# Ezreal11/EaBNet

Hardware: AMD Instinct MI355X
Metric: enhanced frames/sec (16 kHz, 8-mic) at 1/2/4/8 MI355X; RTF per utterance (higher is better)
Workload: dtype f32; 1 GPU; BASELINE configs[1]/[2]: batch of 16 four-second 8-mic 16 kHz utterances per GPU, wave -> STFT+compress -> EaBNet.forward, inference, full hand-written HIP path; batch_per_gpu=16, global_batch=16, mics=8, frames_per_utt=401, freq_bins=161, parallelism=dp1 (independent shards, no collective), pipeline_depth=3

## Files before the change

eabnet_amd/csrc/conv_gemm.hip:

```cpp
#include "device.h"
#include <type_traits>

#define CG_THREADS 256

#define CG_PLAIN 0
#define CG_GLU 1
#define CG_DUAL 2
#define CG_PH2 3
#define CG_XFC 128

#define CG_PMAX 352

template <int MI, int NI, int KU, int MODE, bool PATCH>
struct CgSmem {
    static constexpr int BM = 64 * MI, BN = 64 * NI, LDK = 16 * KU + 4;
    static constexpr int NA = MODE == CG_DUAL ? 2 : 1;
    static constexpr int ATILE = BM * LDK;
    float a[PATCH ? CG_PMAX * LDK : NA * 2 * ATILE];
    float b[2][BN * LDK];
    float xft[2][CG_XFC][2];
    float xsl[2][CG_XFC];
    int dt[EAB_MAX_TAPS];
    int ioff[EAB_MAX_TAPS];
    int last;
};

__device__ __forceinline__ void cg_merge(float& n, float& mean, float& m2, float nb, float meanb, float m2b) {
    const float nt = n + nb;
    if (nt > 0.0f) {
        const float delta = meanb - mean;
        const float fb = nb / nt;
        mean = fmaf(delta, fb, mean);
        m2 = m2 + m2b + delta * delta * n * fb;
    }
    n = nt;
}

template <int MI, int NI, int KU, int MODE, int XF, bool VEC, int PREC, bool PATCH, bool WIDE = false>
__global__ __launch_bounds__(CG_THREADS, (MI == 2 && NI == 2 && KU == 1 && MODE == CG_GLU) ? 3 : (MODE == CG_PH2 ? 2 : 1)) void conv_gemm_kernel(const eab_conv_desc d) {
    static_assert(MODE != CG_PH2 || (PATCH && NI == 2), "phase-pair form: patch pipeline, one column block per phase and wave");
    static_assert(!PATCH || (KU == 1 && MODE != CG_DUAL && VEC), "patch mode: one unit per stage, single transform");
    constexpr bool H3 = PREC == EAB_PREC_F16X3;
    constexpr bool BF = PREC == EAB_PREC_BF16;
    constexpr bool PH2 = MODE == CG_PH2;
    constexpr bool GLU = MODE != CG_PLAIN;
    constexpr bool DUAL = MODE == CG_DUAL;
    using Smem = CgSmem<MI, NI, KU, MODE, PATCH>;
    constexpr int BM = Smem::BM, BN = Smem::BN, LDK = Smem::LDK;
    __shared__ __attribute__((aligned(16))) Smem sm;

    const int tid = threadIdx.x;
    const int lane = tid & 63, wave = tid >> 6;
    const int wm = wave >> 1, wn = wave & 1;
    const int li = lane & 31, lh = lane >> 5;

    const int t_lo = d.win.pos ? *d.win.pos : 0;
    int t_hi = d.win.pos ? (t_lo + d.win.count < d.T ? t_lo + d.win.count : d.T) : d.T;
    const int tiles_per_b = ((d.win.pos ? d.win.count : d.T) * d.No + BM - 1) / BM;
    unsigned vblk = blockIdx.x;
    if (gridDim.x >= 64) {
        const unsigned G = gridDim.x, G8 = G >> 3, rem = G & 7, xcd = vblk & 7, idx = vblk >> 3;
        vblk = xcd * G8 + (xcd < rem ? xcd : rem) + idx;
    }
    const int b = (int)(vblk / (unsigned)tiles_per_b);
    const int tile = (int)vblk - b * tiles_per_b;
    if (d.win.lens) t_hi = min(t_hi, d.win.lens[b]);
    const int Q = t_hi * d.No;
    const int q0 = t_lo * d.No + tile * BM;
    const int n_blk = blockIdx.y * BN;
    const float inv_no = 1.0f / (float)d.No;

#pragma unroll
    for (int j = 0; j < EAB_MAX_TAPS; ++j)
        if (tid == j) {
            sm.dt[j] = d.dt[j];
            sm.ioff[j] = d.ioff[j];
        }

    if (XF != EAB_XF_NONE) {
        const int k = tid >> 7, c = tid & (CG_XFC - 1);
        const int Ck = (k == 0 || DUAL) ? d.C0 : d.C1;
        const float* xfk = k == 0 ? d.xf0 : d.xf1;
        const float* slk = k == 0 ? d.slope0 : d.slope1;
        float sc = 1.0f, sh = 0.0f, sl = 1.0f;
        if (c < Ck) {
            if (d.fin_stats && k < d.fin_nsets) {
                const float* gm = k == 0 ? d.fin_gamma0 : d.fin_gamma1;
                const float* bt = k == 0 ? d.fin_beta0 : d.fin_beta1;
                double sn = 0.0, sm = 0.0, sq = 0.0;
                for (int t = 0; t < d.fin_tiles; ++t) {
                    const f32x4 v = *reinterpret_cast<const f32x4*>(
                        &d.fin_stats[((((size_t)b * d.fin_tiles + t) * d.fin_nsets + k) * d.C0 + c) * 4]);
                    const double n = (double)v[0], mu = (double)v[1];
                    sn += n;
                    sm = fma(n, mu, sm);
                    sq += fma(n * mu, mu, (double)v[2]);
                }
                const double mean = sn > 0.0 ? sm / sn : 0.0;
                double var = sn > 0.0 ? sq / sn - mean * mean : 0.0;
                if (var < 0.0) var = 0.0;
                const double scale = (double)gm[c] / sqrt(var + (double)d.fin_eps);
                sc = (float)scale;
                sh = (float)((double)bt[c] - mean * scale);
                sl = slk[c];
            } else if (xfk) {
                const float2 v = *reinterpret_cast<const float2*>(&xfk[((size_t)b * Ck + c) * 2]);
                sc = v.x;
                sh = v.y;
                sl = slk[c];
            }
        }
        sm.xft[k][c][0] = sc;
        sm.xft[k][c][1] = sh;
        sm.xsl[k][c] = sl;
    }

    const int Ctot = d.C0 + d.C1;
    const int UPT = (Ctot + 15) >> 4;
    const int NU = d.ntaps * UPT;
    static_assert(!WIDE || (PREC == EAB_PREC_BF16 && KU == 1 && VEC && !PATCH && XF == EAB_XF_NONE && MODE != CG_DUAL), "WIDE: see above");
    constexpr bool w0 = WIDE, w1 = WIDE;
    const int NS = (w0 || w1) ? d.ntaps * ((w0 ? d.C0 >> 5 : (d.C0 + 15) >> 4) + (d.C1 > 0 ? (w1 ? d.C1 >> 5 : (d.C1 + 15) >> 4) : 0))
                              : (NU + KU - 1) / KU;

    constexpr unsigned esz0 = WIDE ? 2u : 4u, esz1 = WIDE ? 2u : 4u;
    const unsigned bytes0 = (unsigned)d.T * d.Fin * d.C0 * esz0;
    const unsigned bytes1 = (unsigned)d.T * d.Fin * d.C1 * esz1;
    const __amdgpu_buffer_rsrc_t rs0 = __builtin_amdgcn_make_buffer_rsrc(
        const_cast<char*>(reinterpret_cast<const char*>(d.src0)) + (size_t)b * bytes0, 0, bytes0, 0x00020000);
    const __amdgpu_buffer_rsrc_t rs1 = __builtin_amdgcn_make_buffer_rsrc(
        const_cast<char*>(reinterpret_cast<const char*>(d.src1 ? d.src1 : d.src0)) + (d.src1 ? (size_t)b * bytes1 : 0), 0,
        d.src1 ? bytes1 : 0u, 0x00020000);

    const int srow = tid >> 2;
    const int skq = tid & 3;
    int a_t[MI], a_f0[MI], a_tf[MI];
    bool a_ok[MI];
#pragma unroll
    for (int p = 0; p < MI; ++p) {
        const int q = q0 + srow + 64 * p;
        a_ok[p] = q < Q;
        const int t = a_ok[p] ? eab_div(q, d.No, inv_no) : 0;
        const int o = a_ok[p] ? q - t * d.No : 0;
        a_t[p] = t;
        a_f0[p] = o * d.istride;
        a_tf[p] = t * d.Fin + o * d.istride;
    }
    const float* wrow[NI];
#pragma unroll
    for (int p = 0; p < NI; ++p) wrow[p] = d.w + (size_t)(n_blk + srow + 64 * p) * d.Kpad + skq * 4;

    f32x16 acc[MI][NI];
#pragma unroll
    for (int mi = 0; mi < MI; ++mi)
#pragma unroll
        for (int ni = 0; ni < NI; ++ni)
#pragma unroll
            for (int r = 0; r < 16; ++r) acc[mi][ni][r] = 0.0f;

    auto lds_barrier = [] { asm volatile("s_waitcnt lgkmcnt(0)\n\ts_barrier" ::: "memory"); };

    __syncthreads();

    if (q0 < Q) {
    if constexpr (PATCH) {
        constexpr int PP = (CG_PMAX + 63) / 64;
        int dt_min = 0, io_min = 0, io_max = 0;
#pragma unroll
        for (int j = 0; j < EAB_MAX_TAPS; ++j)
            if (j < d.ntaps) {
                dt_min = d.dt[j] < dt_min ? d.dt[j] : dt_min;
                io_min = d.ioff[j] < io_min ? d.ioff[j] : io_min;
                io_max = d.ioff[j] > io_max ? d.ioff[j] : io_max;
            }
        const int halo_lo = -io_min;
        const int hi_need = (d.No - 1) * d.istride + io_max - (d.Fin - 1);
        const int Fp = d.Fin + halo_lo + (hi_need > 0 ? hi_need : 0);
        const float inv_fp = 1.0f / (float)Fp;
        const int t_first = eab_div(q0, d.No, inv_no);
        const int t_last = eab_div((q0 + BM < Q ? q0 + BM : (Q > q0 ? Q : q0 + 1)) - 1, d.No, inv_no);
        const int P = (t_last - t_first + 1 - dt_min) * Fp;

        int p_tf[PP];
        bool p_ok[PP];
#pragma unroll
        for (int pp = 0; pp < PP; ++pp) {
            const int pidx = srow + 64 * pp;
            const int tr = eab_div(pidx, Fp, inv_fp);
            const int t_in = t_first + dt_min + tr, fi = pidx - tr * Fp - halo_lo;
            p_ok[pp] = pidx < P && t_in >= 0 && t_in < d.T && fi >= 0 && fi < d.Fin;
            p_tf[pp] = t_in * d.Fin + fi;
        }
        int fa[MI];
#pragma unroll
        for (int mi = 0; mi < MI; ++mi) {
            int q = q0 + (wm * MI + mi) * 32 + li;
            q = q < Q ? q : (Q > q0 ? Q - 1 : q0);
            const int t = eab_div(q, d.No, inv_no), o = q - t * d.No;
            fa[mi] = ((t - t_first - dt_min) * Fp + o * d.istride + halo_lo) * LDK + 4 * lh;
        }
        const int b_base = (wn * NI * 32 + li) * LDK + 4 * lh;

        f32x4 rp[PP];
        f32x4 rbw0[NI], rbw1[NI];
        int p_tc = 0;
        auto patch_fetch = [&](int chunk) {
            const int c0 = chunk << 4;
            const bool second = (d.C1 > 0) && (c0 >= d.C0);
            const int Cs = second ? d.C1 : d.C0;
            const int c = (second ? c0 - d.C0 : c0) + skq * 4;
            const bool cok = c < Cs;
            p_tc = ((second ? 1 : 0) << 8) | (cok ? c : 0);
#pragma unroll
            for (int pp = 0; pp < PP; ++pp) {
                const unsigned off = (p_ok[pp] && cok) ? (unsigned)((p_tf[pp] * Cs + c) * 4) : EAB_OOB;
                const u32x4 v = second ? __builtin_amdgcn_raw_buffer_load_b128(rs1, off, 0, 0)
                                       : __builtin_amdgcn_raw_buffer_load_b128(rs0, off, 0, 0);
                rp[pp] = __builtin_bit_cast(f32x4, v);
            }
        };
        auto patch_stash = [&]() {
            f32x4 sh01, sh23, sl;
            if (XF != EAB_XF_NONE) {
                const int cc = p_tc & 0xFF, tb = p_tc >> 8;
                sh01 = *reinterpret_cast<const f32x4*>(&sm.xft[tb][cc][0]);
                sh23 = *reinterpret_cast<const f32x4*>(&sm.xft[tb][cc + 2][0]);
                sl = *reinterpret_cast<const f32x4*>(&sm.xsl[tb][cc]);
            }
#pragma unroll
            for (int pp = 0; pp < PP; ++pp) {
                const int pidx = srow + 64 * pp;
                if (pidx >= CG_PMAX) continue;
                f32x4 v = rp[pp];
                if (XF != EAB_XF_NONE) {
                    const f32x4 x = eab_xform<XF>(v, sh01, sh23, sl);
                    v = p_ok[pp] ? x : f32x4{0.f, 0.f, 0.f, 0.f};
                }
                float* arow = &sm.a[pidx * LDK];
                if (BF) {
                    *reinterpret_cast<uint2*>(reinterpret_cast<char*>(arow) + skq * 8) = make_uint2(eab_bf2(v[0], v[1]), eab_bf2(v[2], v[3]));
                } else if (H3) {
                    unsigned h01, l01, h23, l23;
                    eab_split2(v[0], v[1], h01, l01);
                    eab_split2(v[2], v[3], h23, l23);
                    *reinterpret_cast<uint2*>(reinterpret_cast<char*>(arow) + skq * 8) = make_uint2(h01, h23);
                    *reinterpret_cast<uint2*>(reinterpret_cast<char*>(arow) + 32 + skq * 8) = make_uint2(l01, l23);
                } else {
                    *reinterpret_cast<f32x4*>(arow + skq * 4) = v;
                }
            }
        };
        auto b_fetch = [&](int u, f32x4 (&rbw)[NI]) {
            const int uu = u < NU ? u : 0;
#pragma unroll
            for (int p = 0; p < NI; ++p) rbw[p] = *reinterpret_cast<const f32x4*>(wrow[p] + (size_t)uu * 16);
        };
        auto b_stash = [&](int buf, const f32x4 (&rbw)[NI]) {
#pragma unroll
            for (int p = 0; p < NI; ++p) {
                float* brow = &sm.b[buf][(srow + 64 * p) * LDK];
                if (BF) {
                    *reinterpret_cast<uint2*>(reinterpret_cast<char*>(brow) + skq * 8) =
                        make_uint2(eab_bf2(rbw[p][0], rbw[p][1]), eab_bf2(rbw[p][2], rbw[p][3]));
                } else if (H3) {
                    const u32x4 w = __builtin_bit_cast(u32x4, rbw[p]);
                    *reinterpret_cast<uint2*>(reinterpret_cast<char*>(brow) + skq * 8) = make_uint2(w[0], w[1]);
                    *reinterpret_cast<uint2*>(reinterpret_cast<char*>(brow) + 32 + skq * 8) = make_uint2(w[2], w[3]);
                } else {
                    *reinterpret_cast<f32x4*>(brow + skq * 4) = rbw[p];
                }
            }
        };
        auto pcompute_n = [&](int cur, int tap, auto ne_c) {
            constexpr int NE = decltype(ne_c)::value;
            const int toff = (sm.dt[tap] * Fp + sm.ioff[tap]) * LDK;
            if (BF) {
                bf16x8 ab[MI], bb[NE];
#pragma unroll
                for (int mi = 0; mi < MI; ++mi) ab[mi] = *reinterpret_cast<const bf16x8*>(&sm.a[fa[mi] + toff]);
#pragma unroll
                for (int ni = 0; ni < NE; ++ni) bb[ni] = *reinterpret_cast<const bf16x8*>(&sm.b[cur][b_base + ni * 32 * LDK]);
#pragma unroll
                for (int mi = 0; mi < MI; ++mi)
#pragma unroll
                    for (int ni = 0; ni < NE; ++ni)
                        acc[mi][ni] = __builtin_amdgcn_mfma_f32_32x32x16_bf16(ab[mi], bb[ni], acc[mi][ni], 0, 0, 0);
            } else if (H3) {
                h16x8 ah[MI], al[MI], bh[NE], bl[NE];
#pragma unroll
                for (int mi = 0; mi < MI; ++mi) {
                    const char* pa = reinterpret_cast<const char*>(&sm.a[fa[mi] + toff]);
                    ah[mi] = *reinterpret_cast<const h16x8*>(pa);
                    al[mi] = *reinterpret_cast<const h16x8*>(pa + 32);
                }
#pragma unroll
                for (int ni = 0; ni < NE; ++ni) {
                    const char* pb = reinterpret_cast<const char*>(&sm.b[cur][b_base + ni * 32 * LDK]);
                    bh[ni] = *reinterpret_cast<const h16x8*>(pb);
                    bl[ni] = *reinterpret_cast<const h16x8*>(pb + 32);
                }
#pragma unroll
                for (int mi = 0; mi < MI; ++mi)
#pragma unroll
                    for (int ni = 0; ni < NE; ++ni) {
                        acc[mi][ni] = __builtin_amdgcn_mfma_f32_32x32x16_f16(al[mi], bh[ni], acc[mi][ni], 0, 0, 0);
                        acc[mi][ni] = __builtin_amdgcn_mfma_f32_32x32x16_f16(ah[mi], bl[ni], acc[mi][ni], 0, 0, 0);
                        acc[mi][ni] = __builtin_amdgcn_mfma_f32_32x32x16_f16(ah[mi], bh[ni], acc[mi][ni], 0, 0, 0);
                    }
            } else {
#pragma unroll
                for (int g = 0; g < 2; ++g) {
                    f32x4 af[MI], bf[NE];
#pragma unroll
                    for (int mi = 0; mi < MI; ++mi) af[mi] = *reinterpret_cast<const f32x4*>(&sm.a[fa[mi] + toff + g * 8]);
#pragma unroll
                    for (int ni = 0; ni < NE; ++ni)
                        bf[ni] = *reinterpret_cast<const f32x4*>(&sm.b[cur][b_base + ni * 32 * LDK + g * 8]);
#pragma unroll
                    for (int k = 0; k < 4; ++k)
#pragma unroll
                        for (int mi = 0; mi < MI; ++mi)
#pragma unroll
                            for (int ni = 0; ni < NE; ++ni)
                                acc[mi][ni] = __builtin_amdgcn_mfma_f32_32x32x2f32(af[mi][k], bf[ni][k], acc[mi][ni], 0, 0, 0);
                }
            }
        };
        const unsigned p2mask = PH2 ? (unsigned)d.p2_mask1 : ~0u;
        auto pcompute = [&](int cur, int tap) {
            if (PH2 && !((p2mask >> tap) & 1u)) pcompute_n(cur, tap, std::integral_constant<int, 1>{});
            else pcompute_n(cur, tap, std::integral_constant<int, NI>{});
        };

        patch_fetch(0);
        b_fetch(0, rbw0);
        patch_stash();
        b_stash(0, rbw0);
        b_fetch(1, rbw0);
        b_fetch(2, rbw1);
        lds_barrier();
        const int pre = d.ntaps >= 3 ? d.ntaps - 3 : 0;
        int chunk = 0, tap = 0;
        auto stage = [&](int u, int cur, f32x4 (&rnext)[NI]) {
            if (tap == pre && chunk + 1 < UPT) patch_fetch(chunk + 1);
            pcompute(cur, tap);
            if (u + 1 < NU) b_stash(cur ^ 1, rnext);
            b_fetch(u + 3, rnext);
            if (tap == d.ntaps - 1 && chunk + 1 < UPT) {
                lds_barrier();
                patch_stash();
            }
            lds_barrier();
            if (++tap == d.ntaps) { tap = 0; ++chunk; }
        };
        for (int u = 0; u < NU; u += 2) {
            stage(u, 0, rbw0);
            if (u + 1 < NU) stage(u + 1, 1, rbw1);
        }
        __syncthreads();
    } else {
    struct Stage {
        f32x4 ra[KU][MI], rb[KU][NI];
        f32x4 rb2[BF ? NI : 1];
        int r_tc[KU];
        bool st_ok[KU][MI];
    };
    Stage sa;

    bool tap_ok[MI];
    unsigned tap_b0[MI], tap_b1[MI];
#pragma unroll
    for (int p = 0; p < MI; ++p) {
        tap_ok[p] = false;
        tap_b0[p] = tap_b1[p] = 0u;
    }
    int g_tap = -1, g_c0 = 0, g_w = 16;
    constexpr bool LEAN = KU == 1 && VEC && !DUAL;
    const __amdgpu_buffer_rsrc_t rsw = __builtin_amdgcn_make_buffer_rsrc(const_cast<float*>(d.w), 0, (unsigned)d.N * d.Kpad * 4u, 0x00020000);
    unsigned w_off[NI];
#pragma unroll
    for (int p = 0; p < NI; ++p) w_off[p] = (unsigned)((n_blk + srow + 64 * p) * d.Kpad + skq * 4) * 4u;
    auto fetch = [&](int stage, Stage& rg) {
        if constexpr (LEAN) {
            if (stage == 0) {
                g_tap = 0;
                g_c0 = 0;
            } else {
                g_c0 += g_w;
                if (g_c0 >= (UPT << 4)) {
                    g_c0 = 0;
                    ++g_tap;
                }
            }
            if (g_c0 == 0) {
                const int dt = sm.dt[g_tap], io = sm.ioff[g_tap];
#pragma unroll
                for (int p = 0; p < MI; ++p) {
                    const int tt = a_t[p] + dt, fi = a_f0[p] + io;
                    tap_ok[p] = a_ok[p] && tt >= 0 && tt < d.T && fi >= 0 && fi < d.Fin;
                    const unsigned pos = (unsigned)(a_tf[p] + dt * d.Fin + io);
                    tap_b0[p] = (pos * (unsigned)d.C0 + (unsigned)(skq * (w0 ? 8 : 4))) * esz0;
                    tap_b1[p] = (pos * (unsigned)d.C1 + (unsigned)(skq * (w1 ? 8 : 4))) * esz1;
                }
            }
            const bool second = (d.C1 > 0) && (g_c0 >= d.C0);
            const int Cs = second ? d.C1 : d.C0;
            const int cu = second ? g_c0 - d.C0 : g_c0;
            constexpr bool half = WIDE;
            g_w = half ? 32 : 16;
            const bool cok = cu + skq * (half ? 8 : 4) < Cs;
            const int k0 = g_tap * (UPT << 4) + g_c0;
#pragma unroll
            for (int p = 0; p < MI; ++p) {
                const bool ok = tap_ok[p] && cok;
                rg.st_ok[0][p] = ok;
                const unsigned off = ok ? (second ? tap_b1[p] : tap_b0[p]) : EAB_OOB;
                const u32x4 v = second ? __builtin_amdgcn_raw_buffer_load_b128(rs1, off, cu * (half ? 2 : 4), 0)
                                       : __builtin_amdgcn_raw_buffer_load_b128(rs0, off, cu * (half ? 2 : 4), 0);
                rg.ra[0][p] = __builtin_bit_cast(f32x4, v);
            }
            rg.r_tc[0] = ((half ? 1 : 0) << 9) | ((second ? 1 : 0) << 8) | cu;
#pragma unroll
            for (int p = 0; p < NI; ++p) {
                if constexpr (WIDE) {
                    rg.rb[0][p] = __builtin_bit_cast(f32x4, __builtin_amdgcn_raw_buffer_load_b128(rsw, w_off[p] + skq * 16, k0 * 4, 0));
                    if constexpr (BF)
                        rg.rb2[p] = __builtin_bit_cast(f32x4, __builtin_amdgcn_raw_buffer_load_b128(rsw, w_off[p] + skq * 16, k0 * 4 + 16, 0));
                } else {
                    rg.rb[0][p] = __builtin_bit_cast(f32x4, __builtin_amdgcn_raw_buffer_load_b128(rsw, w_off[p], k0 * 4, 0));
                }
            }
            return;
        }
#pragma unroll
        for (int ku = 0; ku < KU; ++ku) {
            const int u = stage * KU + ku;
            const bool live = u < NU;
            if (u == 0) {
                g_tap = 0;
                g_c0 = 0;
            } else if (live) {
                g_c0 += 16;
                if (g_c0 >= (UPT << 4)) {
                    g_c0 = 0;
                    ++g_tap;
                }
            }
            const int uu = live ? u : 0;
            const int c0 = live ? g_c0 : 0;
            if (live && c0 == 0) {
                const int dt = sm.dt[g_tap], io = sm.ioff[g_tap];
#pragma unroll
                for (int p = 0; p < MI; ++p) {
                    const int tt = a_t[p] + dt, fi = a_f0[p] + io;
                    tap_ok[p] = a_ok[p] && tt >= 0 && tt < d.T && fi >= 0 && fi < d.Fin;
                    const unsigned pos = (unsigned)(a_tf[p] + dt * d.Fin + io);
                    tap_b0[p] = pos * (unsigned)(d.C0 * 4);
                    tap_b1[p] = pos * (unsigned)(d.C1 * 4);
                }
            }
            const bool second = (d.C1 > 0) && (c0 >= d.C0);
            const int Cs = second ? d.C1 : d.C0;
            const int c = (second ? c0 - d.C0 : c0) + skq * 4;
            const bool cok = live && (c < Cs);
#pragma unroll
            for (int p = 0; p < MI; ++p) {
                const bool ok = tap_ok[p] && cok;
                rg.st_ok[ku][p] = ok;
                const unsigned off = ok ? (second ? tap_b1[p] : tap_b0[p]) + (unsigned)(c * 4) : EAB_OOB;
                if (VEC) {
                    const u32x4 v = second ? __builtin_amdgcn_raw_buffer_load_b128(rs1, off, 0, 0)
                                           : __builtin_amdgcn_raw_buffer_load_b128(rs0, off, 0, 0);
                    rg.ra[ku][p] = __builtin_bit_cast(f32x4, v);
                } else {
#pragma unroll
                    for (int j = 0; j < 4; ++j) {
                        const unsigned oj = (ok && c + j < Cs) ? off + 4u * j : EAB_OOB;
                        const unsigned v = second ? __builtin_amdgcn_raw_buffer_load_b32(rs1, oj, 0, 0)
                                                  : __builtin_amdgcn_raw_buffer_load_b32(rs0, oj, 0, 0);
                        rg.ra[ku][p][j] = __builtin_bit_cast(float, v);
                    }
                }
            }
            rg.r_tc[ku] = ((second ? 1 : 0) << 8) | (cok ? c : 0);
#pragma unroll
            for (int p = 0; p < NI; ++p) {
                rg.rb[ku][p] = *reinterpret_cast<const f32x4*>(wrow[p] + (size_t)uu * 16);
                if (!live) rg.rb[ku][p] = f32x4{0.f, 0.f, 0.f, 0.f};
            }
        }
    };

    auto stash = [&](int buf, const Stage& rg) {
#pragma unroll
        for (int ku = 0; ku < KU; ++ku) {
            f32x4 sh01[2], sh23[2], sl[2];
            bool all_ok = false;
            if (XF != EAB_XF_NONE) {
                if constexpr (LEAN) {
                    const int tb = (rg.r_tc[ku] >> 8) & 1, cu = rg.r_tc[ku] & 0xFF;
                    const char* px = reinterpret_cast<const char*>(&sm.xft[0][skq * 4][0]) + (tb * CG_XFC + cu) * 8;
                    const char* ps = reinterpret_cast<const char*>(&sm.xsl[0][skq * 4]) + (tb * CG_XFC + cu) * 4;
                    sh01[0] = *reinterpret_cast<const f32x4*>(px);
                    sh23[0] = *reinterpret_cast<const f32x4*>(px + 16);
                    sl[0] = *reinterpret_cast<const f32x4*>(ps);
                    bool ok_all = true;
#pragma unroll
                    for (int p = 0; p < MI; ++p) ok_all = ok_all && rg.st_ok[ku][p];
                    all_ok = __builtin_amdgcn_ballot_w64(ok_all) == __builtin_amdgcn_ballot_w64(true);
                } else {
                const int cc = rg.r_tc[ku] & 0xFF;
#pragma unroll
                for (int k = 0; k < (DUAL ? 2 : 1); ++k) {
// ... 24 lines not shown
                        else
                            *reinterpret_cast<uint2*>(reinterpret_cast<char*>(arow) + skq * 8) = make_uint2(eab_bf2(v[0], v[1]), eab_bf2(v[2], v[3]));
                    } else if (H3) {
                        unsigned h01, l01, h23, l23;
                        eab_split2(v[0], v[1], h01, l01);
                        eab_split2(v[2], v[3], h23, l23);
                        *reinterpret_cast<uint2*>(reinterpret_cast<char*>(arow) + skq * 8) = make_uint2(h01, h23);
                        *reinterpret_cast<uint2*>(reinterpret_cast<char*>(arow) + 32 + skq * 8) = make_uint2(l01, l23);
                    } else {
                        *reinterpret_cast<f32x4*>(arow + skq * 4) = v;
                    }
                }
            }
#pragma unroll
            for (int p = 0; p < NI; ++p) {
                float* brow = &sm.b[buf][(srow + 64 * p) * LDK + ku * 16];
                if (BF) {
                    if constexpr (WIDE) {
                        const f32x4 r0 = rg.rb[ku][p], r1 = rg.rb2[BF ? p : 0];
                        *reinterpret_cast<u32x4*>(reinterpret_cast<char*>(brow) + skq * 16) =
                            u32x4{eab_bf2(r0[0], r0[1]), eab_bf2(r0[2], r0[3]), eab_bf2(r1[0], r1[1]), eab_bf2(r1[2], r1[3])};
                    } else {
                        *reinterpret_cast<uint2*>(reinterpret_cast<char*>(brow) + skq * 8) =
                            make_uint2(eab_bf2(rg.rb[ku][p][0], rg.rb[ku][p][1]), eab_bf2(rg.rb[ku][p][2], rg.rb[ku][p][3]));
                    }
                } else if (H3) {
                    const u32x4 w = __builtin_bit_cast(u32x4, rg.rb[ku][p]);
                    *reinterpret_cast<uint2*>(reinterpret_cast<char*>(brow) + skq * 8) = make_uint2(w[0], w[1]);
                    *reinterpret_cast<uint2*>(reinterpret_cast<char*>(brow) + 32 + skq * 8) = make_uint2(w[2], w[3]);
                } else {
                    *reinterpret_cast<f32x4*>(brow + skq * 4) = rg.rb[ku][p];
                }
            }
        }
    };

    fetch(0, sa);
    stash(0, sa);
    lds_barrier();

    const int a_base = (wm * MI * 32 + li) * LDK + 4 * lh;
    const int b_base = (wn * NI * 32 + li) * LDK + 4 * lh;

    auto compute = [&](int cur) {
        if (BF) {
#pragma unroll
            for (int ku = 0; ku < KU; ++ku) {
                bf16x8 ab[Smem::NA][MI], bb[NI];
#pragma unroll
                for (int k = 0; k < Smem::NA; ++k)
#pragma unroll
                    for (int mi = 0; mi < MI; ++mi)
                        ab[k][mi] = *reinterpret_cast<const bf16x8*>(&sm.a[(k * 2 + cur) * Smem::ATILE + a_base + mi * 32 * LDK + ku * 16]);
#pragma unroll
                for (int ni = 0; ni < NI; ++ni) bb[ni] = *reinterpret_cast<const bf16x8*>(&sm.b[cur][b_base + ni * 32 * LDK + ku * 16]);
#pragma unroll
                for (int mi = 0; mi < MI; ++mi)
#pragma unroll
                    for (int ni = 0; ni < NI; ++ni)
                        acc[mi][ni] = __builtin_amdgcn_mfma_f32_32x32x16_bf16(ab[DUAL ? ni : 0][mi], bb[ni], acc[mi][ni], 0, 0, 0);
            }
            if constexpr (WIDE) {
                bf16x8 ab[MI], bb[NI];
#pragma unroll
                for (int mi = 0; mi < MI; ++mi) ab[mi] = *reinterpret_cast<const bf16x8*>(&sm.a[cur * Smem::ATILE + a_base + mi * 32 * LDK + 8]);
#pragma unroll
                for (int ni = 0; ni < NI; ++ni) bb[ni] = *reinterpret_cast<const bf16x8*>(&sm.b[cur][b_base + ni * 32 * LDK + 8]);
#pragma unroll
                for (int mi = 0; mi < MI; ++mi)
#pragma unroll
                    for (int ni = 0; ni < NI; ++ni)
                        acc[mi][ni] = __builtin_amdgcn_mfma_f32_32x32x16_bf16(ab[mi], bb[ni], acc[mi][ni], 0, 0, 0);
            }
        } else if (H3) {
#pragma unroll
            for (int ku = 0; ku < KU; ++ku) {
                h16x8 ah[Smem::NA][MI], al[Smem::NA][MI], bh[NI], bl[NI];
#pragma unroll
                for (int k = 0; k < Smem::NA; ++k)
#pragma unroll
                    for (int mi = 0; mi < MI; ++mi) {
                        const char* pa = reinterpret_cast<const char*>(&sm.a[(k * 2 + cur) * Smem::ATILE + a_base + mi * 32 * LDK + ku * 16]);
                        ah[k][mi] = *reinterpret_cast<const h16x8*>(pa);
                        al[k][mi] = *reinterpret_cast<const h16x8*>(pa + 32);
                    }
#pragma unroll
                for (int ni = 0; ni < NI; ++ni) {
                    const char* pb = reinterpret_cast<const char*>(&sm.b[cur][b_base + ni * 32 * LDK + ku * 16]);
                    bh[ni] = *reinterpret_cast<const h16x8*>(pb);
                    bl[ni] = *reinterpret_cast<const h16x8*>(pb + 32);
                }
#pragma unroll
                for (int mi = 0; mi < MI; ++mi)
#pragma unroll
                    for (int ni = 0; ni < NI; ++ni) {
                        const int ka = DUAL ? ni : 0;
                        acc[mi][ni] = __builtin_amdgcn_mfma_f32_32x32x16_f16(al[ka][mi], bh[ni], acc[mi][ni], 0, 0, 0);
                        acc[mi][ni] = __builtin_amdgcn_mfma_f32_32x32x16_f16(ah[ka][mi], bl[ni], acc[mi][ni], 0, 0, 0);
                        acc[mi][ni] = __builtin_amdgcn_mfma_f32_32x32x16_f16(ah[ka][mi], bh[ni], acc[mi][ni], 0, 0, 0);
                    }
            }
        } else {
#pragma unroll
        for (int g = 0; g < 2 * KU; ++g) {
            f32x4 af[Smem::NA][MI], bf[NI];
#pragma unroll
            for (int k = 0; k < Smem::NA; ++k)
#pragma unroll
                for (int mi = 0; mi < MI; ++mi)
                    af[k][mi] = *reinterpret_cast<const f32x4*>(&sm.a[(k * 2 + cur) * Smem::ATILE + a_base + mi * 32 * LDK + g * 8]);
#pragma unroll
            for (int ni = 0; ni < NI; ++ni)
                bf[ni] = *reinterpret_cast<const f32x4*>(&sm.b[cur][b_base + ni * 32 * LDK + g * 8]);
#pragma unroll
            for (int k = 0; k < 4; ++k)
#pragma unroll
                for (int mi = 0; mi < MI; ++mi)
#pragma unroll
                    for (int ni = 0; ni < NI; ++ni)
                        acc[mi][ni] = __builtin_amdgcn_mfma_f32_32x32x2f32(af[DUAL ? ni : 0][mi][k], bf[ni][k],
                                                                           acc[mi][ni], 0, 0, 0);
        }
        }
    };
    constexpr bool PF2 = MI * NI <= 2 && KU == 1 && MODE == CG_PLAIN;
    if constexpr (PF2) {
        Stage sb;
        if (NS > 1) fetch(1, sb);
        for (int s = 0; s < NS; s += 2) {
            if (s + 2 < NS) fetch(s + 2, sa);
            compute(0);
            if (s + 1 < NS) stash(1, sb);
            lds_barrier();
            if (s + 1 < NS) {
                if (s + 3 < NS) fetch(s + 3, sb);
                compute(1);
                if (s + 2 < NS) stash(0, sa);
                lds_barrier();
            }
        }
    } else {
    for (int s = 0; s < NS; ++s) {
        const int cur = s & 1;
        if (s + 1 < NS) fetch(s + 1, sa);
        compute(cur);
        if (s + 1 < NS) stash(cur ^ 1, sa);
        lds_barrier();
    }
    }

    }
    }

    constexpr int NC = GLU ? 1 : NI;
    const int Cout = d.Cout;
    int ch[NC];
    float bias_v[NI];
#pragma unroll
    for (int ni = 0; ni < NI; ++ni) {
        const int n = n_blk + (wn * NI + ni) * 32 + li;
        bias_v[ni] = d.bias ? d.bias[n] : 0.0f;
    }
    if (GLU) {
        ch[0] = (n_blk >> 1) + wn * 32 + li;
    } else {
#pragma unroll
        for (int ni = 0; ni < NI; ++ni) ch[ni] = n_blk + (wn * NI + ni) * 32 + li;
    }
    float st_slope[2][NC];
#pragma unroll
    for (int s = 0; s < 2; ++s)
#pragma unroll
        for (int c = 0; c < NC; ++c) {
            const float* sp = s == 0 ? d.stat_slope0 : d.stat_slope1;
            st_slope[s][c] = (d.stats && s < d.nsets && sp) ? sp[ch[c]] : 1.0f;
        }
    float skk[2][NC], ssum[2][NC], ssq[2][NC];
    float scount = 0.0f;
#pragma unroll
    for (int s = 0; s < 2; ++s)
#pragma unroll
        for (int c = 0; c < NC; ++c) skk[s][c] = ssum[s][c] = ssq[s][c] = 0.0f;
    const bool two_sets = d.nsets == 2;
    const unsigned out_bytes = (unsigned)d.T * d.Fout * Cout * 4u;
    const size_t out_b = (size_t)b * d.T * d.Fout * Cout;
    const bool need_aux = d.epi == EAB_EPI_MULSIG || d.epi == EAB_EPI_ADD;
    const __amdgpu_buffer_rsrc_t r_dst = __builtin_amdgcn_make_buffer_rsrc(d.dst + out_b, 0, out_bytes, 0x00020000);
    const __amdgpu_buffer_rsrc_t r_aux = __builtin_amdgcn_make_buffer_rsrc(
        const_cast<float*>(need_aux ? d.aux + out_b : d.dst + out_b), 0, need_aux ? out_bytes : 0u, 0x00020000);
    const __amdgpu_buffer_rsrc_t r_acc = __builtin_amdgcn_make_buffer_rsrc(
        d.dst_acc ? d.dst_acc + out_b : d.dst + out_b, 0, d.dst_acc ? out_bytes : 0u, 0x00020000);

    const unsigned row_bytes = (unsigned)(d.Fout * Cout) * 4u, step_bytes = (unsigned)(d.ostride * Cout) * 4u;
    const unsigned phase_bytes = (unsigned)(d.ophase * Cout) * 4u;
    if constexpr (PH2) {
        const float a = st_slope[0][0];
        const float k0 = eab_prelu(acc[0][0][0] + bias_v[0], a);
        const unsigned chan_bytes = (unsigned)Cout * 4u;
        float su = 0.0f, sq = 0.0f, cnt = 0.0f;
        auto ph2_loop = [&](auto full_c) {
            constexpr bool FULL = decltype(full_c)::value;
#pragma unroll
            for (int mi = 0; mi < MI; ++mi) {
#pragma unroll
                for (int r4 = 0; r4 < 4; ++r4) {
                    const int qg = q0 + (wm * MI + mi) * 32 + 8 * r4 + 4 * lh;
                    const int t = eab_div((FULL || qg < Q) ? qg : 0, d.No, inv_no);
                    int o = ((FULL || qg < Q) ? qg : 0) - t * d.No;
                    unsigned row_start = (unsigned)t * row_bytes;
                    unsigned cur = row_start + (unsigned)o * step_bytes;
#pragma unroll
                    for (int j = 0; j < 4; ++j) {
                        const int r = 4 * r4 + j;
                        const bool ok0 = FULL || qg + j < Q;
                        const bool ok1 = ok0 && 2 * o + 1 < d.Fout;
                        const float v0 = acc[mi][0][r] + bias_v[0], v1 = acc[mi][1][r] + bias_v[1];
                        const unsigned o0 = cur + 4u * ch[0];
                        __builtin_amdgcn_raw_buffer_store_b32(__builtin_bit_cast(unsigned, v0), r_dst, ok0 ? o0 : EAB_OOB, 0, 0);
                        __builtin_amdgcn_raw_buffer_store_b32(__builtin_bit_cast(unsigned, v1), r_dst, ok1 ? o0 + chan_bytes : EAB_OOB, 0, 0);
                        const float e0 = eab_prelu(v0, a) - k0, e1 = eab_prelu(v1, a) - k0;
                        const float m0 = FULL ? e0 : (ok0 ? e0 : 0.0f), m1 = ok1 ? e1 : 0.0f;
                        su += m0;
                        sq = fmaf(m0, m0, sq);
                        su += m1;
                        sq = fmaf(m1, m1, sq);
                        cnt += (FULL ? 1.0f : (ok0 ? 1.0f : 0.0f)) + (ok1 ? 1.0f : 0.0f);
                        cur += step_bytes;
                        if (++o == d.No) {
                            o = 0;
                            row_start += row_bytes;
                            cur = row_start;
                        }
                    }
                }
            }
        };
        if (q0 + BM <= Q) ph2_loop(std::true_type{});
        else ph2_loop(std::false_type{});
        skk[0][0] = k0;
        ssum[0][0] = su;
        ssq[0][0] = sq;
        scount = cnt;
    } else {
    const bool fast_epi = !DUAL && q0 + BM <= Q && d.dst_acc == nullptr && !two_sets &&
                          (GLU ? true : (d.epi == EAB_EPI_LINEAR || d.epi == EAB_EPI_ADD));
    if (fast_epi) {
        auto fast_loop = [&](auto dump_c, auto add_c) {
            constexpr bool DUMPV = decltype(dump_c)::value, ADDV = decltype(add_c)::value;
#pragma unroll
            for (int mi = 0; mi < MI; ++mi) {
                unsigned off[16];
#pragma unroll
                for (int r4 = 0; r4 < 4; ++r4) {
                    const int qg = q0 + (wm * MI + mi) * 32 + 8 * r4 + 4 * lh;
                    const int t = eab_div(qg, d.No, inv_no);
                    int o = qg - t * d.No;
                    unsigned row_start = (unsigned)t * row_bytes + phase_bytes;
                    unsigned cur = row_start + (unsigned)o * step_bytes;
#pragma unroll
                    for (int j = 0; j < 4; ++j) {
                        off[4 * r4 + j] = cur;
                        cur += step_bytes;
                        if (++o == d.No) {
                            o = 0;
                            row_start += row_bytes;
                            cur = row_start;
                        }
                    }
                }
                float auxv[16][NC];
                if (ADDV) {
#pragma unroll
                    for (int r = 0; r < 16; ++r)
#pragma unroll
                        for (int c = 0; c < NC; ++c)
                            auxv[r][c] = __builtin_bit_cast(float, __builtin_amdgcn_raw_buffer_load_b32(r_aux, off[r] + 4u * ch[c], 0, 0));
                }
#pragma unroll
                for (int r = 0; r < 16; ++r) {
#pragma unroll
                    for (int c = 0; c < NC; ++c) {
                        float v;
                        if constexpr (GLU) {
                            const float av = acc[mi][0][r] + bias_v[0], sv = eab_fast_sigmoid(acc[mi][1][r] + bias_v[1]);
                            v = av * sv;
                            if (DUMPV) {
                                float* dp = d.glu_dump + 2 * (out_b + (off[r] >> 2)) + n_blk + wn * 64 + li;
                                dp[0] = av;
                                dp[32] = sv;
                            }
                        } else {
                            v = acc[mi][c][r] + bias_v[c];
                        }
                        if (ADDV) v = v + auxv[r][c];
                        __builtin_amdgcn_raw_buffer_store_b32(__builtin_bit_cast(unsigned, v), r_dst, off[r] + 4u * ch[c], 0, 0);
                        acc[mi][c][r] = v;
                    }
                }
            }
        };
        const bool dump = GLU && d.glu_dump != nullptr, add = !GLU && d.epi == EAB_EPI_ADD;
        if (dump) fast_loop(std::true_type{}, std::false_type{});
        else if (add) fast_loop(std::false_type{}, std::true_type{});
        else fast_loop(std::false_type{}, std::false_type{});
        if (d.stats) {
#pragma unroll
            for (int c = 0; c < NC; ++c) {
                const float a = st_slope[0][c];
                const float k0 = eab_prelu(acc[0][c][0], a);
                float su = 0.0f, sq = 0.0f;
#pragma unroll
                for (int mi = 0; mi < MI; ++mi)
#pragma unroll
                    for (int r = 0; r < 16; ++r) {
                        const float e = eab_prelu(acc[mi][c][r], a) - k0;
                        su += e;
                        sq = fmaf(e, e, sq);
                    }
                skk[0][c] = k0;
                ssum[0][c] = su;
                ssq[0][c] = sq;
            }
            scount = (float)(16 * MI);
        }
    } else
#pragma unroll
    for (int mi = 0; mi < MI; ++mi) {
        unsigned off[16];
        bool rowok[16];
#pragma unroll
        for (int r4 = 0; r4 < 4; ++r4) {
            const int qg = q0 + (wm * MI + mi) * 32 + 8 * r4 + 4 * lh;
            const int t = eab_div(qg < Q ? qg : 0, d.No, inv_no);
            int o = (qg < Q ? qg : 0) - t * d.No;
            unsigned row_start = (unsigned)t * row_bytes + phase_bytes;
            unsigned cur = row_start + (unsigned)o * step_bytes;
#pragma unroll
            for (int j = 0; j < 4; ++j) {
                const int r = 4 * r4 + j;
                rowok[r] = qg + j < Q;
                off[r] = rowok[r] ? cur : EAB_OOB;
                cur += step_bytes;
                if (++o == d.No) {
                    o = 0;
                    row_start += row_bytes;
                    cur = row_start;
                }
            }
        }
        float auxv[16][NC], accv[16][NC];
        if (need_aux) {
#pragma unroll
            for (int r = 0; r < 16; ++r)
#pragma unroll
                for (int c = 0; c < NC; ++c)
                    auxv[r][c] = __builtin_bit_cast(float, __builtin_amdgcn_raw_buffer_load_b32(
                                                               r_aux, rowok[r] ? off[r] + 4u * ch[c] : EAB_OOB, 0, 0));
        }
        if (d.dst_acc) {
#pragma unroll
            for (int r = 0; r < 16; ++r)
#pragma unroll
                for (int c = 0; c < NC; ++c)
                    accv[r][c] = __builtin_bit_cast(float, __builtin_amdgcn_raw_buffer_load_b32(
                                                               r_acc, rowok[r] ? off[r] + 4u * ch[c] : EAB_OOB, 0, 0));
        }
#pragma unroll
        for (int r = 0; r < 16; ++r) {
#pragma unroll
            for (int c = 0; c < NC; ++c) {
                float v;
                if (GLU) {
                    const float av = acc[mi][0][r] + bias_v[0], sv = eab_fast_sigmoid(acc[mi][1][r] + bias_v[1]);
                    v = av * sv;
                    if (d.glu_dump && rowok[r]) {
                        float* dp = d.glu_dump + 2 * (out_b + (off[r] >> 2)) + n_blk + wn * 64 + li;
                        dp[0] = av;
                        dp[32] = sv;
                    }
                } else {
                    v = acc[mi][c][r] + bias_v[c];
                }
                if (d.epi == EAB_EPI_RELU) v = fmaxf(v, 0.0f);
                else if (d.epi == EAB_EPI_MULSIG) v = auxv[r][c] * eab_fast_sigmoid(v);
                else if (d.epi == EAB_EPI_ADD) v = v + auxv[r][c];
                const unsigned o4 = rowok[r] ? off[r] + 4u * ch[c] : EAB_OOB;
                __builtin_amdgcn_raw_buffer_store_b32(__builtin_bit_cast(unsigned, v), r_dst, o4, 0, 0);
                if (d.dst_acc)
                    __builtin_amdgcn_raw_buffer_store_b32(__builtin_bit_cast(unsigned, v + accv[r][c]), r_acc, o4, 0, 0);
                if (rowok[r]) {
                    const bool first = scount == 0.0f;
                    const float g0 = eab_prelu(v, st_slope[0][c]);
                    if (first) skk[0][c] = g0;
                    const float e0 = g0 - skk[0][c];
                    ssum[0][c] += e0;
                    ssq[0][c] = fmaf(e0, e0, ssq[0][c]);
                    if (two_sets) {
                        const float g1 = eab_prelu(v, st_slope[1][c]);
                        if (first) skk[1][c] = g1;
                        const float e1 = g1 - skk[1][c];
                        ssum[1][c] += e1;
                        ssq[1][c] = fmaf(e1, e1, ssq[1][c]);
                    }
                }
            }
            if (rowok[r]) scount += 1.0f;
        }
    }

    }
    if (d.stats) {
        float* red = &sm.a[0];
        float mean[2][NC], m2[2][NC];
        float cnt = scount;
        const float inv_n = scount > 0.0f ? 1.0f / scount : 0.0f;
#pragma unroll
        for (int s = 0; s < 2; ++s)
#pragma unroll
            for (int c = 0; c < NC; ++c) {
                mean[s][c] = fmaf(ssum[s][c], inv_n, skk[s][c]);
                m2[s][c] = fmaxf(ssq[s][c] - ssum[s][c] * ssum[s][c] * inv_n, 0.0f);
            }
        const float cnt_o = __shfl_xor(cnt, 32);
#pragma unroll
        for (int s = 0; s < 2; ++s)
#pragma unroll
            for (int c = 0; c < NC; ++c) {
                float n = cnt;
                const float mo = __shfl_xor(mean[s][c], 32), qo = __shfl_xor(m2[s][c], 32);
                if (lh == 0) cg_merge(n, mean[s][c], m2[s][c], cnt_o, mo, qo);
            }
        cnt += cnt_o;
        if (lh == 0) {
#pragma unroll
            for (int s = 0; s < 2; ++s)
#pragma unroll
                for (int c = 0; c < NC; ++c) {
                    const int i = ((((wm * 2 + wn) * 2 + s) * NC + c) * 32 + li) * 3;
                    red[i] = cnt;
                    red[i + 1] = mean[s][c];
                    red[i + 2] = m2[s][c];
                }
        }
        __syncthreads();
        if (wm == 0 && lh == 0) {
            const size_t tbase = ((size_t)b * d.stat_tiles + d.stat_tile0 + tile) * d.nsets;
#pragma unroll
            for (int s = 0; s < 2; ++s) {
                if (s >= d.nsets) break;
#pragma unroll
                for (int c = 0; c < NC; ++c) {
                    const int i0 = ((((0 * 2 + wn) * 2 + s) * NC + c) * 32 + li) * 3;
                    const int i1 = ((((1 * 2 + wn) * 2 + s) * NC + c) * 32 + li) * 3;
                    float n = red[i0], mu = red[i0 + 1], q = red[i0 + 2];
                    cg_merge(n, mu, q, red[i1], red[i1 + 1], red[i1 + 2]);
                    *reinterpret_cast<f32x4*>(&d.stats[((tbase + s) * Cout + ch[c]) * 4]) = f32x4{n, mu, q, 0.0f};
                }
            }
        }
        if (d.fz_counter) {
            __threadfence();
            __syncthreads();
            if (tid == 0) sm.last = atomicAdd(&d.fz_counter[b], 1) == d.stat_tiles - 1;
            __syncthreads();
            if (sm.last) {
                __threadfence();
                const int nch = d.nsets * Cout;
                const int NSL = CG_THREADS / nch;
                const int e = tid % nch, slice = tid / nch;
                const int s = e / Cout, c = e - s * Cout;
                double* dred = reinterpret_cast<double*>(&sm.a[0]);
                double sn = 0.0, sm_ = 0.0, sq = 0.0;
                if (slice < NSL) {
                    const float* p = d.stats + (((size_t)b * d.stat_tiles) * d.nsets + s) * Cout * 4 + (size_t)c * 4;
                    const size_t stride = (size_t)d.nsets * Cout * 4;
                    for (int t = slice; t < d.stat_tiles; t += NSL) {
                        const f32x4 v = *reinterpret_cast<const f32x4*>(p + (size_t)t * stride);
                        const double n = (double)v[0], mu = (double)v[1];
                        sn += n;
                        sm_ = fma(n, mu, sm_);
                        sq += fma(n * mu, mu, (double)v[2]);
                    }
                    dred[(0 * NSL + slice) * nch + e] = sn;
                    dred[(1 * NSL + slice) * nch + e] = sm_;
                    dred[(2 * NSL + slice) * nch + e] = sq;
                }
                __syncthreads();
                if (slice == 0) {
                    sn = sm_ = sq = 0.0;
                    for (int k = 0; k < NSL; ++k) {
                        sn += dred[(0 * NSL + k) * nch + e];
                        sm_ += dred[(1 * NSL + k) * nch + e];
                        sq += dred[(2 * NSL + k) * nch + e];
                    }
                    const double mean = sn > 0.0 ? sm_ / sn : 0.0;
                    double var = sn > 0.0 ? sq / sn - mean * mean : 0.0;
                    if (var < 0.0) var = 0.0;
                    const float* gm = s == 0 ? d.fz_gamma0 : d.fz_gamma1;
                    const float* bt = s == 0 ? d.fz_beta0 : d.fz_beta1;
                    float* xf = s == 0 ? d.fz_xf0 : d.fz_xf1;
                    const double scale = (double)gm[c] / sqrt(var + (double)d.fz_eps);
                    *reinterpret_cast<float2*>(&xf[((size_t)b * Cout + c) * 2]) = make_float2((float)scale, (float)((double)bt[c] - mean * scale));
                }
                if (tid == 0) d.fz_counter[b] = 0;
            }
        }
    }
}

extern "C" int eab_conv_tiles(int T, int No, int bm) {
    if (T <= 0 || No <= 0 || (bm != 16 && bm != 32 && bm != 64 && bm != 128)) return -1;
    long long q = (long long)T * No;
    return (int)((q + bm - 1) / bm);
}

int eab_conv_st(const eab_conv_desc* d, hipStream_t s);

template <int MI, int NI, int KU, int MODE, int XF, bool VEC>
static int cg_launch(const eab_conv_desc* d, hipStream_t s) {
    constexpr int BM = 64 * MI, BN = 64 * NI;
    const int tiles = eab_conv_tiles(d->win.pos ? d->win.count : d->T, d->No, BM);
    dim3 grid((unsigned)(d->B * tiles), (unsigned)(d->N / BN));
    constexpr bool can_patch = KU == 1 && MODE != CG_DUAL && VEC && XF != EAB_XF_PRELU_NORM;
    if (d->korder == EAB_KORDER_CHUNK) {
        if constexpr (can_patch) {
            if (d->precision == EAB_PREC_F16X3)
                hipLaunchKernelGGL((conv_gemm_kernel<MI, NI, 1, MODE, XF, true, EAB_PREC_F16X3, true>), grid,
                                   dim3(CG_THREADS), 0, s, *d);
            else if (d->precision == EAB_PREC_BF16)
                hipLaunchKernelGGL((conv_gemm_kernel<MI, NI, 1, MODE, XF, true, EAB_PREC_BF16, true>), grid,
                                   dim3(CG_THREADS), 0, s, *d);
            else
                hipLaunchKernelGGL((conv_gemm_kernel<MI, NI, 1, MODE, XF, true, EAB_PREC_F32, true>), grid,
                                   dim3(CG_THREADS), 0, s, *d);
            EAB_RETURN_LAUNCH_STATUS();
        } else {
            return EAB_EUNSUPPORTED;
        }
    }
// ... 182 lines not shown
```

Before: 986,400 frames/s.

## Precompute output row offsets in shared table; streamline patch indexing and epilogue

Output row byte offsets are computed once per block into a shared-memory table, reusing the xft buffer when no input transform is active. The epilogues read them with vector LDS loads instead of redoing per-row integer division and wraparound logic. Patch-row index setup becomes incremental instead of a division per slot, and a wave-uniform ballot skips rim masking when a whole wave is in bounds. The PH2 epilogue gains a specialised path when both phase outputs are always valid. This trades extra LDS traffic and a barrier dependency for fewer VALU integer ops and registers. It relies on EAB_OOB offsets being negative when read as signed, and adding the channel offset to them may not stay out of bounds.

Result: faster. 999,900 frames/s, median of 6 (+1.4%).

```diff
diff --git a/eabnet_amd/csrc/conv_gemm.hip b/eabnet_amd/csrc/conv_gemm.hip
--- a/eabnet_amd/csrc/conv_gemm.hip
+++ b/eabnet_amd/csrc/conv_gemm.hip
@@ -11,7 +11,7 @@
 
 #define CG_PMAX 352
 
-template <int MI, int NI, int KU, int MODE, bool PATCH>
+template <int MI, int NI, int KU, int MODE, bool PATCH, bool XFT>
 struct CgSmem {
     static constexpr int BM = 64 * MI, BN = 64 * NI, LDK = 16 * KU + 4;
     static constexpr int NA = MODE == CG_DUAL ? 2 : 1;
@@ -23,6 +23,9 @@
     int dt[EAB_MAX_TAPS];
     int ioff[EAB_MAX_TAPS];
     int last;
+    static constexpr int RW = MODE == CG_PH2 ? 2 : 1;
+    __attribute__((aligned(16))) unsigned rtab_own[XFT ? BM * RW : 4];
+    static_assert(XFT || sizeof(float) * 2 * CG_XFC * 2 >= sizeof(unsigned) * BM * RW, "row table inside xft");
 };
 
 __device__ __forceinline__ void cg_merge(float& n, float& mean, float& m2, float nb, float meanb, float m2b) {
@@ -45,7 +48,7 @@
     constexpr bool PH2 = MODE == CG_PH2;
     constexpr bool GLU = MODE != CG_PLAIN;
     constexpr bool DUAL = MODE == CG_DUAL;
-    using Smem = CgSmem<MI, NI, KU, MODE, PATCH>;
+    using Smem = CgSmem<MI, NI, KU, MODE, PATCH, XF != EAB_XF_NONE>;
     constexpr int BM = Smem::BM, BN = Smem::BN, LDK = Smem::LDK;
     __shared__ __attribute__((aligned(16))) Smem sm;
 
@@ -76,6 +79,21 @@
             sm.dt[j] = d.dt[j];
             sm.ioff[j] = d.ioff[j];
         }
+
+    const int Cout = d.Cout;
+    const unsigned row_bytes = (unsigned)(d.Fout * Cout) * 4u, step_bytes = (unsigned)(d.ostride * Cout) * 4u;
+    const unsigned phase_bytes = (unsigned)(d.ophase * Cout) * 4u, chan_bytes = (unsigned)Cout * 4u;
+    unsigned* const rtab = XF != EAB_XF_NONE ? sm.rtab_own : reinterpret_cast<unsigned*>(&sm.xft[0][0][0]);
+    if (tid < BM) {
+        const int q = q0 + tid;
+        const bool ok = q < Q;
+        const int t = eab_div(ok ? q : 0, d.No, inv_no), o = (ok ? q : 0) - t * d.No;
+        const unsigned off = ok ? (unsigned)t * row_bytes + (unsigned)o * step_bytes + phase_bytes : EAB_OOB;
+        if constexpr (PH2)
+            *reinterpret_cast<uint2*>(&rtab[2 * tid]) = make_uint2(off, (ok && 2 * o + 1 < d.Fout) ? off + chan_bytes : EAB_OOB);
+        else
+            rtab[tid] = off;
+    }
 
     if (XF != EAB_XF_NONE) {
         const int k = tid >> 7, c = tid & (CG_XFC - 1);
@@ -134,18 +152,6 @@
 
     const int srow = tid >> 2;
     const int skq = tid & 3;
-    int a_t[MI], a_f0[MI], a_tf[MI];
-    bool a_ok[MI];
-#pragma unroll
-    for (int p = 0; p < MI; ++p) {
-        const int q = q0 + srow + 64 * p;
-        a_ok[p] = q < Q;
-        const int t = a_ok[p] ? eab_div(q, d.No, inv_no) : 0;
-        const int o = a_ok[p] ? q - t * d.No : 0;
-        a_t[p] = t;
-        a_f0[p] = o * d.istride;
-        a_tf[p] = t * d.Fin + o * d.istride;
-    }
     const float* wrow[NI];
 #pragma unroll
     for (int p = 0; p < NI; ++p) wrow[p] = d.w + (size_t)(n_blk + srow + 64 * p) * d.Kpad + skq * 4;
@@ -181,15 +187,31 @@
         const int t_last = eab_div((q0 + BM < Q ? q0 + BM : (Q > q0 ? Q : q0 + 1)) - 1, d.No, inv_no);
         const int P = (t_last - t_first + 1 - dt_min) * Fp;
 
+        const int d64 = eab_div(64, Fp, inv_fp), m64 = 64 - d64 * Fp;
         int p_tf[PP];
-        bool p_ok[PP];
-#pragma unroll
-        for (int pp = 0; pp < PP; ++pp) {
-            const int pidx = srow + 64 * pp;
-            const int tr = eab_div(pidx, Fp, inv_fp);
-            const int t_in = t_first + dt_min + tr, fi = pidx - tr * Fp - halo_lo;
-            p_ok[pp] = pidx < P && t_in >= 0 && t_in < d.T && fi >= 0 && fi < d.Fin;
-            p_tf[pp] = t_in * d.Fin + fi;
+        bool p_ok[PP], p_all[PP];
+        {
+            const int tr = eab_div(srow, Fp, inv_fp);
+            int f = srow - tr * Fp, t_in = t_first + dt_min + tr;
+            int tf = t_in * d.Fin + f - halo_lo;
+#pragma unroll
+            for (int pp = 0; pp < PP; ++pp) {
+                p_ok[pp] = p_all[pp] = false;
+                p_tf[pp] = 0;
+                if (64 * pp < P) {
+                    p_ok[pp] = srow + 64 * pp < P && (unsigned)t_in < (unsigned)d.T && (unsigned)(f - halo_lo) < (unsigned)d.Fin;
+                    if (XF != EAB_XF_NONE) p_all[pp] = __builtin_amdgcn_ballot_w64(p_ok[pp]) == __builtin_amdgcn_ballot_w64(true);
+                    p_tf[pp] = tf;
+                    f += m64;
+                    t_in += d64;
+                    tf += d64 * d.Fin + m64;
+                    if (f >= Fp) {
+                        f -= Fp;
+                        ++t_in;
+                        tf += d.Fin - Fp;
+                    }
+                }
+            }
         }
         int fa[MI];
 #pragma unroll
@@ -213,6 +235,7 @@
             p_tc = ((second ? 1 : 0) << 8) | (cok ? c : 0);
 #pragma unroll
             for (int pp = 0; pp < PP; ++pp) {
+                if (64 * pp >= P) continue;
                 const unsigned off = (p_ok[pp] && cok) ? (unsigned)((p_tf[pp] * Cs + c) * 4) : EAB_OOB;
                 const u32x4 v = second ? __builtin_amdgcn_raw_buffer_load_b128(rs1, off, 0, 0)
                                        : __builtin_amdgcn_raw_buffer_load_b128(rs0, off, 0, 0);
@@ -231,10 +254,15 @@
             for (int pp = 0; pp < PP; ++pp) {
                 const int pidx = srow + 64 * pp;
                 if (pidx >= CG_PMAX) continue;
+                if (64 * pp >= P) continue;
                 f32x4 v = rp[pp];
                 if (XF != EAB_XF_NONE) {
                     const f32x4 x = eab_xform<XF>(v, sh01, sh23, sl);
-                    v = p_ok[pp] ? x : f32x4{0.f, 0.f, 0.f, 0.f};
+                    v = x;
+                    if (!p_all[pp]) {
+                        asm volatile("; rim" ::: "memory");
+                        v = p_ok[pp] ? x : f32x4{0.f, 0.f, 0.f, 0.f};
+                    }
                 }
                 float* arow = &sm.a[pidx * LDK];
                 if (BF) {
@@ -359,6 +387,18 @@
         }
         __syncthreads();
     } else {
+    int a_t[MI], a_f0[MI], a_tf[MI];
+    bool a_ok[MI];
+#pragma unroll
+    for (int p = 0; p < MI; ++p) {
+        const int q = q0 + srow + 64 * p;
+        a_ok[p] = q < Q;
+        const int t = a_ok[p] ? eab_div(q, d.No, inv_no) : 0;
+        const int o = a_ok[p] ? q - t * d.No : 0;
+        a_t[p] = t;
+        a_f0[p] = o * d.istride;
+        a_tf[p] = t * d.Fin + o * d.istride;
+    }
     struct Stage {
         f32x4 ra[KU][MI], rb[KU][NI];
         f32x4 rb2[BF ? NI : 1];
@@ -689,8 +729,9 @@
     }
     }
 
+    const int rrow = wm * MI * 32 + 4 * lh;
+
     constexpr int NC = GLU ? 1 : NI;
-    const int Cout = d.Cout;
     int ch[NC];
     float bias_v[NI];
 #pragma unroll
@@ -728,52 +769,49 @@
     const __amdgpu_buffer_rsrc_t r_acc = __builtin_amdgcn_make_buffer_rsrc(
         d.dst_acc ? d.dst_acc + out_b : d.dst + out_b, 0, d.dst_acc ? out_bytes : 0u, 0x00020000);
 
-    const unsigned row_bytes = (unsigned)(d.Fout * Cout) * 4u, step_bytes = (unsigned)(d.ostride * Cout) * 4u;
-    const unsigned phase_bytes = (unsigned)(d.ophase * Cout) * 4u;
     if constexpr (PH2) {
         const float a = st_slope[0][0];
         const float k0 = eab_prelu(acc[0][0][0] + bias_v[0], a);
-        const unsigned chan_bytes = (unsigned)Cout * 4u;
-        float su = 0.0f, sq = 0.0f, cnt = 0.0f;
-        auto ph2_loop = [&](auto full_c) {
-            constexpr bool FULL = decltype(full_c)::value;
+        float su = 0.0f, sq = 0.0f;
+        int n1 = 0;
+        const unsigned chb = 4u * ch[0];
+        auto ph2_loop = [&](auto full_c, auto all1_c) {
+            constexpr bool FULL = decltype(full_c)::value, ALL1 = decltype(all1_c)::value;
 #pragma unroll
             for (int mi = 0; mi < MI; ++mi) {
 #pragma unroll
                 for (int r4 = 0; r4 < 4; ++r4) {
-                    const int qg = q0 + (wm * MI + mi) * 32 + 8 * r4 + 4 * lh;
-                    const int t = eab_div((FULL || qg < Q) ? qg : 0, d.No, inv_no);
-                    int o = ((FULL || qg < Q) ? qg : 0) - t * d.No;
-                    unsigned row_start = (unsigned)t * row_bytes;
-                    unsigned cur = row_start + (unsigned)o * step_bytes;
+                    const unsigned* row = &rtab[2 * (rrow + 32 * mi + 8 * r4)];
+                    const u32x4 e[2] = {*reinterpret_cast<const u32x4*>(row), *reinterpret_cast<const u32x4*>(row + 4)};
 #pragma unroll
                     for (int j = 0; j < 4; ++j) {
                         const int r = 4 * r4 + j;
-                        const bool ok0 = FULL || qg + j < Q;
-                        const bool ok1 = ok0 && 2 * o + 1 < d.Fout;
+                        const unsigned t0 = e[j >> 1][2 * (j & 1)], t1 = e[j >> 1][2 * (j & 1) + 1];
+                        const bool ok0 = FULL || (int)t0 >= 0;
+                        const bool ok1 = ALL1 || (int)t1 >= 0;
                         const float v0 = acc[mi][0][r] + bias_v[0], v1 = acc[mi][1][r] + bias_v[1];
-                        const unsigned o0 = cur + 4u * ch[0];
-                        __builtin_amdgcn_raw_buffer_store_b32(__builtin_bit_cast(unsigned, v0), r_dst, ok0 ? o0 : EAB_OOB, 0, 0);
-                        __builtin_amdgcn_raw_buffer_store_b32(__builtin_bit_cast(unsigned, v1), r_dst, ok1 ? o0 + chan_bytes : EAB_OOB, 0, 0);
+                        const unsigned o0 = t0 + chb;
+                        __builtin_amdgcn_raw_buffer_store_b32(__builtin_bit_cast(unsigned, v0), r_dst, o0, 0, 0);
+                        if (ALL1) __builtin_amdgcn_raw_buffer_store_b32(__builtin_bit_cast(unsigned, v1), r_dst, o0, chan_bytes, 0);
+                        else __builtin_amdgcn_raw_buffer_store_b32(__builtin_bit_cast(unsigned, v1), r_dst, t1 + chb, 0, 0);
                         const float e0 = eab_prelu(v0, a) - k0, e1 = eab_prelu(v1, a) - k0;
-                        const float m0 = FULL ? e0 : (ok0 ? e0 : 0.0f), m1 = ok1 ? e1 : 0.0f;
+                        const float m0 = FULL ? e0 : (ok0 ? e0 : 0.0f), m1 = ALL1 ? e1 : (ok1 ? e1 : 0.0f);
                         su += m0;
                         sq = fmaf(m0, m0, sq);
                         su += m1;
                         sq = fmaf(m1, m1, sq);
-                        cnt += (FULL ? 1.0f : (ok0 ? 1.0f : 0.0f)) + (ok1 ? 1.0f : 0.0f);
-                        cur += step_bytes;
-                        if (++o == d.No) {
-                            o = 0;
-                            row_start += row_bytes;
-                            cur = row_start;
-                        }
+                        if (!FULL) n1 += ok0 ? 1 : 0;
+                        if (!ALL1) n1 += ok1 ? 1 : 0;
                     }
                 }
             }
         };
-        if (q0 + BM <= Q) ph2_loop(std::true_type{});
-        else ph2_loop(std::false_type{});
+        const bool full = q0 + BM <= Q;
+        const bool all1 = full && d.Fout == 2 * d.No;
+        if (all1) ph2_loop(std::true_type{}, std::true_type{});
+        else if (full) ph2_loop(std::true_type{}, std::false_type{});
+        else ph2_loop(std::false_type{}, std::false_type{});
+        const float cnt = (float)((full ? 16 * MI : 0) + (all1 ? 16 * MI : 0) + n1);
         skk[0][0] = k0;
         ssum[0][0] = su;
         ssq[0][0] = sq;
@@ -789,21 +827,9 @@
                 unsigned off[16];
 #pragma unroll
                 for (int r4 = 0; r4 < 4; ++r4) {
-                    const int qg = q0 + (wm * MI + mi) * 32 + 8 * r4 + 4 * lh;
-                    const int t = eab_div(qg, d.No, inv_no);
-                    int o = qg - t * d.No;
-                    unsigned row_start = (unsigned)t * row_bytes + phase_bytes;
-                    unsigned cur = row_start + (unsigned)o * step_bytes;
-#pragma unroll
-                    for (int j = 0; j < 4; ++j) {
-                        off[4 * r4 + j] = cur;
-                        cur += step_bytes;
-                        if (++o == d.No) {
-                            o = 0;
-                            row_start += row_bytes;
-                            cur = row_start;
-                        }
-                    }
+                    const u32x4 e = *reinterpret_cast<const u32x4*>(&rtab[rrow + 32 * mi + 8 * r4]);
+#pragma unroll
+                    for (int j = 0; j < 4; ++j) off[4 * r4 + j] = e[j];
                 }
                 float auxv[16][NC];
                 if (ADDV) {
@@ -867,22 +893,11 @@
         bool rowok[16];
 #pragma unroll
         for (int r4 = 0; r4 < 4; ++r4) {
-            const int qg = q0 + (wm * MI + mi) * 32 + 8 * r4 + 4 * lh;
-            const int t = eab_div(qg < Q ? qg : 0, d.No, inv_no);
-            int o = (qg < Q ? qg : 0) - t * d.No;
-            unsigned row_start = (unsigned)t * row_bytes + phase_bytes;
-            unsigned cur = row_start + (unsigned)o * step_bytes;
+            const u32x4 e = *reinterpret_cast<const u32x4*>(&rtab[rrow + 32 * mi + 8 * r4]);
 #pragma unroll
             for (int j = 0; j < 4; ++j) {
-                const int r = 4 * r4 + j;
-                rowok[r] = qg + j < Q;
-                off[r] = rowok[r] ? cur : EAB_OOB;
-                cur += step_bytes;
-                if (++o == d.No) {
-                    o = 0;
-                    row_start += row_bytes;
-                    cur = row_start;
-                }
+                off[4 * r4 + j] = e[j];
+                rowok[4 * r4 + j] = (int)e[j] >= 0;
             }
         }
         float auxv[16][NC], accv[16][NC];
@@ -892,7 +907,7 @@
 #pragma unroll
                 for (int c = 0; c < NC; ++c)
                     auxv[r][c] = __builtin_bit_cast(float, __builtin_amdgcn_raw_buffer_load_b32(
-                                                               r_aux, rowok[r] ? off[r] + 4u * ch[c] : EAB_OOB, 0, 0));
+                                                               r_aux, off[r] + 4u * ch[c], 0, 0));
         }
         if (d.dst_acc) {
 #pragma unroll
@@ -900,7 +915,7 @@
 #pragma unroll
                 for (int c = 0; c < NC; ++c)
                     accv[r][c] = __builtin_bit_cast(float, __builtin_amdgcn_raw_buffer_load_b32(
-                                                               r_acc, rowok[r] ? off[r] + 4u * ch[c] : EAB_OOB, 0, 0));
+                                                               r_acc, off[r] + 4u * ch[c], 0, 0));
         }
 #pragma unroll
         for (int r = 0; r < 16; ++r) {
@@ -921,7 +936,7 @@
                 if (d.epi == EAB_EPI_RELU) v = fmaxf(v, 0.0f);
                 else if (d.epi == EAB_EPI_MULSIG) v = auxv[r][c] * eab_fast_sigmoid(v);
                 else if (d.epi == EAB_EPI_ADD) v = v + auxv[r][c];
-                const unsigned o4 = rowok[r] ? off[r] + 4u * ch[c] : EAB_OOB;
+                const unsigned o4 = off[r] + 4u * ch[c];
                 __builtin_amdgcn_raw_buffer_store_b32(__builtin_bit_cast(unsigned, v), r_dst, o4, 0, 0);
                 if (d.dst_acc)
                     __builtin_amdgcn_raw_buffer_store_b32(__builtin_bit_cast(unsigned, v + accv[r][c]), r_acc, o4, 0, 0);
```
